# populationgenomics/cuKING

Hardware: AMD Instinct MI355X
Metric: sample-pairs/s (all-pairs KING) (higher is better)
Workload: dtype fp4 products, f32 accumulate (exact integers)

## Files before the change

### cuking_amd/_lib.py

```python
from __future__ import annotations

import ctypes as C
from pathlib import Path

PKG = Path(__file__).resolve().parent
LIB_PATH = PKG / "libcuking_amd.so"

OK = 0
ERR_INVALID_ARGUMENT = 1
ERR_FAILED_PRECONDITION = 2
ERR_RESOURCE_EXHAUSTED = 3
ERR_OUT_OF_MEMORY = 4
ERR_DEVICE = 5

KERNEL_TILED = 0
KERNEL_STREAM = 1

KIN_UPPER = 0
KIN_SYMMETRIC = 1

KIN_BINS_MAX = 4096
REL_THRESHOLDS_MAX = 8
REL_NO_BAND = 0xFFFFFFFF

# ... 108 lines not shown
    "cuking_kin_best_key": (_u64, [_f32, _u32]),
    "cuking_kin_best_decode": (_u32, [_u64, C.POINTER(_f32), C.POINTER(_u32)]),
    "cuking_compute_kin_summary": (_int, [_vp, _SM, _u32, _vp, _BINS, _vp, _vp, _vp]),
    "cuking_compute_kin_summary_tiles": (_int, [_vp, _SM, _u32, _vp, _u64, _u64, _BINS, _vp,
                                                _vp, _vp]),
    "cuking_rel_band": (_u32, [C.POINTER(_f32), _u32, _f32]),
    "cuking_compute_relative_counts": (_int, [_vp, _SM, _u32, _vp, C.POINTER(_f32), _u32, _vp,
                                              _vp]),
    "cuking_compute_relative_counts_tiles": (_int, [_vp, _SM, _u32, _vp, _u64, _u64,
                                                    C.POINTER(_f32), _u32, _vp, _vp]),
    "cuking_unrelated_key": (_u64, [_f32, _u32]),
    "cuking_unrelated_set_host": (_int, [_vp, _u64, _u32, _f32, _vp, _vp, _vp]),
    "cuking_unrelated_set": (_int, [_vp, _vp, _u64, _u32, _f32, _vp, _vp, _vp, C.POINTER(_u32),
                                    _vp]),
    "cuking_site_counts": (_int, [_vp, _vp, _u32, _u32, _vp, _vp]),
    "cuking_sample_counts": (_int, [_vp, _vp, _u32, _u32, _u32, _vp, _vp]),
    "cuking_site_mask_host": (_int, [_vp, _u32, _u32, C.POINTER(CSiteFilter), _vp, _vp,
                                     C.POINTER(_u32)]),
    "cuking_compact_sites_host": (_int, [_vp, _u32, _u32, _vp, _u32, _vp, _u32]),
    "cuking_compact_sites": (_int, [_vp, _vp, _u32, _u32, _vp, _u32, _vp, _u32, _vp]),
    "cuking_ld_site_words": (_u32, [_u32]),
    "cuking_ld_priority": (_f32, [_vp]),
    "cuking_transpose_sites_host": (_int, [_vp, _u32, _u32, _u32, _vp, _u32]),
    "cuking_transpose_sites": (_int, [_vp, _vp, _u32, _u32, _u32, _vp, _u32, _vp]),
    "cuking_ld_edges_host": (_int, [_vp, _u32, _u32, _u32, _f32, _vp, _vp, _u64,
                                    C.POINTER(_u64)]),
    "cuking_ld_edges": (_int, [_vp, _vp, _u32, _u32, _u32, _f32, _vp, _vp, _u64,
                               C.POINTER(_u64), _vp]),
    "cuking_geno_matmul_host": (_int, [_vp, _u32, _u32, _u32, _vp, _int, _vp, _u32, _u32, _vp,
                                       _u32]),
# ... 89 lines not shown
```

### cuking_amd/build.py

```python
from __future__ import annotations

import argparse
import os
import shutil
import subprocess
import sys
from pathlib import Path

PKG = Path(__file__).resolve().parent
ROOT = PKG.parent
CSRC = PKG / "csrc"
HOST = PKG / "host"
INCLUDE = ROOT / "include"

LIB_PATH = PKG / "libcuking_amd.so"
CLI_PATH = PKG / "bin" / "cuking"
LIB_FLAGS_PATH = PKG / "libcuking_amd.flags"

HIP_SOURCES = ["king_abi.hip", "king_kernels.hip", "king_mfma.hip", "king_filter.hip",
               "king_sort.hip", "king_prune.hip", "king_bed.hip", "king_site_qc.hip",
               "king_ld.hip", "king_geno.hip", "king_pcrelate.hip",
               "king_pcrelate_records.hip", "king_pcrelate_pairs.hip", "king_ibd.hip",
               "king_ibd_scan.hip", "king_mendel.hip", "synth.hip"]
HOST_ABI_SOURCES = ["king_host.cc"]
# ... 38 lines not shown
    cwd = PKG / "build_tmp"
    cwd.mkdir(exist_ok=True)
    cmd += ["-save-temps"]
    if save_temps:
        cmd += ["-Rpass-analysis=kernel-resource-usage"]
        subprocess.run(cmd, check=True, cwd=str(cwd))
    else:
        with open(cwd / "build.log", "w") as log:
            r = subprocess.run(cmd, cwd=str(cwd), stdout=log, stderr=subprocess.STDOUT)
        if r.returncode != 0:
            sys.stderr.write((cwd / "build.log").read_text()[-8000:])
            raise subprocess.CalledProcessError(r.returncode, cmd)
    problems = check_mfma_loops(cwd / "king_mfma-hip-amdgcn-amd-amdhsa-gfx950.s")
    problems += check_filter_loop(cwd / "king_filter-hip-amdgcn-amd-amdhsa-gfx950.s")
    problems += check_no_scratch(cwd / "king_bed-hip-amdgcn-amd-amdhsa-gfx950.s", "pack_bed_kernel")
    for kernel in ("site_counts_kernel", "sample_counts_kernel", "compact_sites_kernel"):
        problems += check_no_scratch(cwd / "king_site_qc-hip-amdgcn-amd-amdhsa-gfx950.s", kernel)
    for kernel in ("transpose_sites_kernel", "ld_edges_kernel"):
        problems += check_no_scratch(cwd / "king_ld-hip-amdgcn-amd-amdhsa-gfx950.s", kernel)
    problems += check_no_scratch(cwd / "king_geno-hip-amdgcn-amd-amdhsa-gfx950.s",
                                 "geno_matmul_kernel")
    problems += check_no_scratch(cwd / "king_pcrelate-hip-amdgcn-amd-amdhsa-gfx950.s",
                                 "pcrelate_matrix_kernel")
    problems += check_no_scratch(cwd / "king_pcrelate_records-hip-amdgcn-amd-amdhsa-gfx950.s",
                                 "pcrelate_records_kernel")
    problems += check_no_scratch(cwd / "king_pcrelate_pairs-hip-amdgcn-amd-amdhsa-gfx950.s",
                                 "pcrelate_pairs_kernel")
    for kernel in ("ibd_pairs_kernel", "roh_samples_kernel"):
        problems += check_no_scratch(cwd / "king_ibd-hip-amdgcn-amd-amdhsa-gfx950.s", kernel)
    problems += check_no_scratch(cwd / "king_ibd_scan-hip-amdgcn-amd-amdhsa-gfx950.s",
# ... 128 lines not shown
```

### cuking_amd/csrc/king_abi.hip

```cpp
#include <hip/hip_runtime.h>

#include <algorithm>
#include <cstdio>
#include <cstdlib>
#include <cstring>
#include <vector>

#include "king_common.h"
#include "king_geno.h"
#include "king_host.h"
#include "king_ibd.h"
#include "king_kin_summary.h"
#include "king_ld.h"
#include "king_site_qc.h"
#include "king_unrelated.h"

using namespace cuking;

namespace {

#define HIP_TRY(expr)                                                      \
  do {                                                                     \
    const hipError_t _e = (expr);                                          \
    if (_e != hipSuccess) {                                                \
// ... 89 lines not shown
    DeviceBuf prune, sites, record_count, ibd_groups, site_order;
  };
  std::vector<StreamScratch> scratch;
  unsigned long long filter_totals_retired[kNumTotals] = {};
  uint32_t filter_quadrant_cap = kFilterQuadrantCap;
  uint32_t filter_cand_cap = kFilterCandCap;
  uint32_t filter_split_min_steps = 8;
  int filter_check0 = 1, filter_check1 = 1, filter_check_emit = (int)kCheckEmitCap;
  int filter_rotate = 1;
  uint32_t filter_rotate_min_steps = 128;
  uint32_t filter_rotate_min_tiles = 2048;
  int filter_sort = 1;
  bool filter_lazy_codes = true;
  int filter_site_order = -1;
  uint32_t filter_site_order_min_tiles = (uint32_t)kSiteOrderMinTiles;
  SiteOrderForecast order_forecast = {0, 0, false};
  float order_sigma = 0.f;
  void *sort_temp = nullptr;
  size_t sort_temp_bytes = 0;

  void *synth_tables = nullptr;
  size_t synth_tables_bytes = 0;
  hipStream_t synth_stream = nullptr;
  hipEvent_t synth_done = nullptr;

  struct Prepared {
    bool valid = false;
    cuking_submatrix sm = {0, 0, 0, 0};
    uint32_t words_per_sample = 0;
    int variant = -1;
// ... 476 lines not shown
  const uint32_t all_tiles = (geo.s_stride + 63) / 64;
  const uint32_t t_end = s_tile_end < all_tiles ? s_tile_end : all_tiles;
  cuking_ctx::Prepared &pr = ctx->prepared;
  const bool new_prefix = !same_tile_space(ctx->prefix_for, tiles);
  const uint32_t num_stored = geo.diag ? geo.num_rows : geo.num_rows + geo.num_cols;
  SiteOrderScratch order_layout = {};
  bool order_wanted = false;
  if (filter_call && !dense_order && v.layout == kLayoutNibbleStats && ctx->filter_site_order != 0 &&
      s_tile_begin == 0 && t_end == all_tiles) {
    order_layout = site_order_scratch(num_stored, words_per_sample);
    order_wanted = order_layout.bytes != 0 &&
                 (ctx->filter_site_order >= 1 ||
                  (total_tiles(tiles) >= ctx->filter_site_order_min_tiles &&
                   geo.k_words / 8 >= filter_check_min_steps()));
  }
  const bool same = same_block(pr, sm, words_per_sample, variant, v.tile, d_bit_sets) &&
                    pr.dense_order == dense_order && pr.order_wanted == order_wanted &&
                    !(pr.site_order && pr.order_thr != kin_threshold);
  if (ctx->reuse_prepared && same && !new_prefix) {
    bool all_there = true;
    for (uint32_t t = s_tile_begin; t < t_end && all_there; ++t) all_there = pr.tiles[t] != 0;
    if (all_there) {
      ++ctx->conversions_skipped;
      if (v.layout == kLayoutNibbleStats && need_codes && !pr.codes)
        return convert_codes_now(ctx, geo, words_per_sample, d_bit_sets, stream);
      return CUKING_OK;
    }
  }
  const bool other_stream = pr.ordered_valid && pr.ordered_on != stream;
  bool must_wait = new_prefix && !ctx->readers.empty();
// ... 49 lines not shown
                                order_layout, d_curve, stream));
      SiteCurve curve;
      HIP_TRY(hipMemcpyAsync(&curve, d_curve, sizeof curve, hipMemcpyDeviceToHost, stream));
      ++ctx->host_syncs;
      HIP_TRY(hipStreamSynchronize(stream));
      const SiteOrderForecast f = site_order_forecast(curve, num_stored, geo.k_words, kin_threshold);
      ctx->order_forecast = f;
      ctx->order_sigma = curve.sigma;
      site_order = ctx->filter_site_order >= 1 ||
                   (!f.verdict_first && f.order64 != 0 &&
                    (f.stored64 == 0 || f.order64 + kSiteOrderMinGain <= f.stored64));
      pr.order_thr = kin_threshold;
      pr.order_no_left = site_order ? 0u : kSiteOrderNoTrust;
    }
    pr.site_order = site_order;
    if (site_order) {
      cuking_ctx::StreamScratch *e = stream_entry(ctx, stream);
      HIP_TRY(launch_site_permute(d_bit_sets, num_stored, words_per_sample, e->site_order.p,
                                  order_layout, stream));
      layout_bits = reinterpret_cast<const uint64_t *>(static_cast<const uint8_t *>(e->site_order.p) +
                                                       order_layout.permuted);
    }
    HIP_TRY(launch_sample_stats(layout_bits, words_per_sample, geo, ctx->planes, sb, se, stream));
    HIP_TRY(launch_sample_order(geo, words_per_sample, ctx->planes, sb, se,
                                !dense_order &&
                                    (ctx->filter_sort == 2 || (ctx->filter_sort == 1 && whole)),
                                ctx->sort_temp, ctx->sort_temp_bytes, stream));
    HIP_TRY(launch_prepare_nibbles(codes && !site_order, true, layout_bits, words_per_sample, geo,
                                   ctx->planes, plane_perm(ctx->planes, geo), s_tile_begin, t_end,
                                   nullptr, nullptr, stream));
    if (codes && site_order)
      HIP_TRY(launch_prepare_nibbles(true, false, d_bit_sets, words_per_sample, geo, ctx->planes,
                                     plane_perm(ctx->planes, geo), s_tile_begin, t_end, nullptr,
                                     nullptr, stream));
    if (!codes) {
      pr.codes = false;
    } else if (!pr.codes) {
      st = convert_codes_now(ctx, geo, words_per_sample, d_bit_sets, stream);
// ... 88 lines not shown

enum : uint8_t {
  kInvalidatesLayout = 1,
  kResizesSlabs = 2,
};

struct Option {
  const char *key;
  int64_t lo, hi;
  const char *error;
  uint32_t error_arg;
  uint8_t effects;
  int64_t (*get)(const cuking_ctx *);
  void (*set)(cuking_ctx *, int64_t);
  int64_t hole = INT64_MIN;
};

#define CTX_FIELD(f)                                                     \
  [](const cuking_ctx *c) -> int64_t { return (int64_t)c->f; },          \
  [](cuking_ctx *c, int64_t v) { c->f = (decltype(c->f))v; }

const Option kOptions[] = {
    {"variant", 0, kNumTiledVariants - 1, "variant outside [0, %u)", kNumTiledVariants, 0,
     CTX_FIELD(variant)},
    {"band_rows", 0, 64, "band_rows outside [0, 64]", 0, 0, CTX_FIELD(band_rows)},
    {"counts_mode", -1, 1, "counts_mode outside [-1, 1]", 0, 0, CTX_FIELD(counts_mode)},
    {"split_wgs", 0, 4096, "split_wgs outside [0, 4096]", 0, kResizesSlabs, CTX_FIELD(split_wgs)},
    {"xcd_swizzle", 0, 2, "xcd_swizzle outside [0, 2]", 0, 0, CTX_FIELD(xcd_swizzle)},
    {"dyn_tail_tiles", 0, 0x7FFFFFFF, "dyn_tail_tiles outside [0, 2^31)", 0, 0,
     CTX_FIELD(dyn_tail_tiles)},
    {"reuse_prepared", 0, 1, "reuse_prepared outside [0, 1]", 0, 0, CTX_FIELD(reuse_prepared)},
    {"filter_sort", 0, 2, "filter_sort outside [0, 2]", 0, kInvalidatesLayout,
     CTX_FIELD(filter_sort)},
    {"filter_lazy_codes", 0, 1, "filter_lazy_codes outside [0, 1]", 0, kInvalidatesLayout,
     CTX_FIELD(filter_lazy_codes)},
    {"filter_site_order", -1, 2, "filter_site_order outside [-1, 2]", 0, kInvalidatesLayout,
     CTX_FIELD(filter_site_order)},
    {"filter_site_order_min_tiles", 0, 1 << 30, "filter_site_order_min_tiles outside [0, 2^30]",
     0, kInvalidatesLayout, CTX_FIELD(filter_site_order_min_tiles)},
    {"filter_check0", 0, 2, "filter_check0 outside [0, 2]", 0, 0, CTX_FIELD(filter_check0)},
    {"filter_check1", 0, 1 + kNumCheckShares, "filter_check1 outside {0, 1, 3 .. %u}",
     1 + kNumCheckShares, 0, CTX_FIELD(filter_check1), 2},
    {"filter_check_emit", 0, 255, "filter_check_emit outside [0, 255]", 0, 0,
     CTX_FIELD(filter_check_emit)},
    {"filter_rotate", 0, 2 + kNumPhases, "filter_rotate outside [0, %u]", 2 + kNumPhases, 0,
     CTX_FIELD(filter_rotate)},
    {"filter_rotate_min_steps", 1, 1 << 20, "filter_rotate_min_steps outside [1, 2^20]", 0, 0,
     CTX_FIELD(filter_rotate_min_steps)},
    {"filter_rotate_min_tiles", 0, 1 << 30, "filter_rotate_min_tiles outside [0, 2^30]", 0, 0,
     CTX_FIELD(filter_rotate_min_tiles)},
    {"filter_quadrant_cap", 0, 16384, "filter_quadrant_cap outside [0, 16384]", 0, 0,
     CTX_FIELD(filter_quadrant_cap)},
    {"filter_cand_cap", 0, kFilterCandCap, "filter_cand_cap outside [0, %u]", kFilterCandCap, 0,
     CTX_FIELD(filter_cand_cap)},
// ... 122 lines not shown

cuking_status cuking_ctx_set_kernel(cuking_ctx *ctx, cuking_kernel kernel) {
  if (ctx == nullptr) return cuking_fail(CUKING_ERR_INVALID_ARGUMENT, "null context");
  if (kernel != CUKING_KERNEL_TILED && kernel != CUKING_KERNEL_STREAM)
    return cuking_fail(CUKING_ERR_INVALID_ARGUMENT, "unknown kernel %d", (int)kernel);
  ctx->kernel = kernel;
  return CUKING_OK;
}

cuking_status cuking_ctx_set_option(cuking_ctx *ctx, const char *key,
                                    int64_t value) {
  if (ctx == nullptr || key == nullptr)
    return cuking_fail(CUKING_ERR_INVALID_ARGUMENT, "null argument");
  const Option *o = find_option(key);
  if (o == nullptr) return cuking_fail(CUKING_ERR_INVALID_ARGUMENT, "unknown option %s", key);
  if (value < o->lo || value > o->hi || value == o->hole)
    return cuking_fail(CUKING_ERR_INVALID_ARGUMENT, o->error, o->error_arg);
  if ((o->effects & kResizesSlabs) && value != o->get(ctx)) {
    HIP_TRY(hipDeviceSynchronize());
    for (auto &e : ctx->scratch) free_split_slab(e);
  }
  o->set(ctx, value);
  if (o->effects & kInvalidatesLayout) ctx->prepared.valid = false;
  return CUKING_OK;
}

cuking_status cuking_device_alloc(cuking_ctx *ctx, size_t bytes, void **d_ptr) {
  BIND_OR_RETURN(ctx);
  if (d_ptr == nullptr) return cuking_fail(CUKING_ERR_INVALID_ARGUMENT, "null out pointer");
  *d_ptr = nullptr;
  if (bytes == 0) return CUKING_OK;
// ... 732 lines not shown

cuking_status cuking_site_counts(cuking_ctx *ctx, const uint64_t *d_bit_set,
                                 uint32_t num_stored, uint32_t words_per_sample,
                                 uint32_t *d_counts, void *stream) {
  if (ctx == nullptr) return cuking_fail(CUKING_ERR_INVALID_ARGUMENT, "null context");
  cuking_status st = cuking_check_counts_args("site counts", d_bit_set, num_stored,
                                              words_per_sample, d_counts);
  if (st != CUKING_OK) return st;
  if (num_stored == 0) return CUKING_OK;
  BIND_OR_RETURN(ctx);
  HIP_TRY(launch_site_counts(d_bit_set, num_stored, words_per_sample, d_counts,
                             (hipStream_t)stream));
  return CUKING_OK;
}

cuking_status cuking_sample_counts(cuking_ctx *ctx, const uint64_t *d_bit_set,
                                   uint32_t num_stored, uint32_t words_per_sample,
                                   uint32_t num_sites, uint32_t *d_counts, void *stream) {
  if (ctx == nullptr) return cuking_fail(CUKING_ERR_INVALID_ARGUMENT, "null context");
  cuking_status st = cuking_check_counts_args("sample counts", d_bit_set, num_stored,
                                              words_per_sample, d_counts);
  if (st != CUKING_OK) return st;
  if (cuking_words_per_sample(num_sites) != words_per_sample)
    return cuking_fail(CUKING_ERR_INVALID_ARGUMENT,
                       "sample counts: %u sites need %u words per sample, not %u", num_sites,
                       cuking_words_per_sample(num_sites), words_per_sample);
  if (num_stored == 0) return CUKING_OK;
  BIND_OR_RETURN(ctx);
  HIP_TRY(launch_sample_counts(d_bit_set, num_stored, words_per_sample, num_sites, d_counts,
                               (hipStream_t)stream));
// ... 406 lines not shown
```

### cuking_amd/csrc/king_common.h

```cpp
#ifndef CUKING_AMD_KING_COMMON_H_
#define CUKING_AMD_KING_COMMON_H_

#include <hip/hip_runtime.h>
#include <stdint.h>

#include "cuking_amd.h"
#include "king_launch_plan.h"
#include "king_submatrix.h"

namespace cuking {

constexpr uint32_t kLayoutWord = 0;
constexpr uint32_t kLayoutQuad = 1;
constexpr uint32_t kLayoutNibble = 2;
constexpr uint32_t kLayoutNibbleStats = 3;

struct PlaneGeometry {
  uint32_t num_rows, num_cols;
  uint32_t rows_padded, cols_padded;
  uint32_t col_base;
  uint32_t s_stride;
  uint32_t k_words;
  uint32_t diag;
};
// ... 267 lines not shown
hipError_t launch_mfma_list(const TiledArgs &args, const uint2 *list, const uint32_t *count,
                            uint32_t cap, uint32_t grid, hipStream_t stream);
hipError_t launch_mfma_gated(const TiledArgs &args, uint64_t num_units, const uint32_t *gate,
                             const uint8_t *skip_tiles, uint64_t skip_base, uint32_t grid,
                             hipStream_t stream);
hipError_t launch_filter(const TiledArgs &args, const LaunchSwitches &sw, uint64_t num_tiles,
                         hipStream_t stream);
inline void to_quadrants(TiledArgs *a, uint64_t *num_units) {
  a->quad = 1;
  a->tile_begin *= 4;
  *num_units *= 4;
}
hipError_t launch_sample_stats(const uint64_t *d_bit_sets, uint32_t words_per_sample,
                               const PlaneGeometry &geo, uint4 *d_planes, uint32_t s_begin,
                               uint32_t s_end, hipStream_t stream);
void set_filter_check_min_steps(uint32_t steps);
uint32_t filter_check_min_steps();
size_t sort_temp_bytes_for(uint32_t n);
hipError_t launch_sample_order(const PlaneGeometry &geo, uint32_t words_per_sample,
                               uint4 *d_planes, uint32_t s_begin, uint32_t s_end, bool sort,
                               void *sort_temp, size_t sort_temp_bytes, hipStream_t stream);
struct SiteOrderScratch {
  size_t counts, keys, vals, sort_temp, sort_temp_bytes, permuted, bytes;
};
SiteOrderScratch site_order_scratch(uint32_t num_stored, uint32_t words_per_sample);
hipError_t launch_site_order(const uint64_t *d_bit_sets, uint32_t num_stored,
                             uint32_t words_per_sample, const PlaneGeometry &geo, void *d_scratch,
                             const SiteOrderScratch &layout, SiteCurve *d_curve,
                             hipStream_t stream);
hipError_t launch_site_permute(const uint64_t *d_bit_sets, uint32_t num_stored,
                               uint32_t words_per_sample, void *d_scratch,
                               const SiteOrderScratch &layout, hipStream_t stream);
struct SiteOrderForecast {
  uint32_t stored64, order64;
  bool verdict_first;
};
SiteOrderForecast site_order_forecast(const SiteCurve &curve, uint32_t num_stored,
                                      uint32_t k_words, float thr);
hipError_t launch_prepare_nibbles(bool codes, bool t2, const uint64_t *d_bit_sets,
                                  uint32_t words_per_sample, const PlaneGeometry &geo,
                                  uint4 *d_planes, const uint32_t *perm, uint32_t s_tile_begin,
                                  uint32_t s_tile_end, const uint32_t *gate,
                                  const uint32_t *ready, hipStream_t stream);
hipError_t launch_mark_codes_ready(const uint32_t *gate, uint32_t *ready, hipStream_t stream);
size_t mfma_split_scratch_bytes(uint32_t wgs);
size_t mfma_split_counter_bytes(uint32_t wgs);

// ... 124 lines not shown
```

### cuking_amd/csrc/king_filter.hip

```cpp
#include <hip/hip_runtime.h>
#include <stdio.h>

#include <atomic>
#include <stdlib.h>

#include "king_common.h"
#include "king_device.h"
#include "king_kin_summary.h"

#pragma clang diagnostic ignored "-Winline-asm"

namespace cuking {

namespace {

typedef int v8i __attribute__((ext_vector_type(8)));
typedef float v16f __attribute__((ext_vector_type(16)));

constexpr int kT = (int)kFilterTile;
constexpr int kUnits = 2;
constexpr int kStages = 5;
constexpr int kSliceU4 = kT;
constexpr int kStageU4 = 2 * 2 * kUnits * kSliceU4;
constexpr int kStageReqs = 4 * kUnits;
// ... 946 lines not shown
        atomicAdd(a.rel_counts + (size_t)off_j * a.rel_num + band, 1u);
      }
    }
  }
}

}

static std::atomic<uint32_t> g_check_min_steps{64};
void set_filter_check_min_steps(uint32_t steps) { g_check_min_steps.store(steps); }
uint32_t filter_check_min_steps() { return g_check_min_steps.load(); }

hipError_t launch_sample_stats(const uint64_t *d_bit_sets, uint32_t words_per_sample,
                               const PlaneGeometry &geo, uint4 *d_planes, uint32_t s_begin,
                               uint32_t s_end, hipStream_t stream) {
  if (s_end > geo.s_stride) s_end = geo.s_stride;
  if (s_begin >= s_end) return hipSuccess;
  float2 *stats = plane_tmp_stats(d_planes, geo);
  float *prefix = plane_tmp_prefix(d_planes, geo);
  unsigned long long *sums = const_cast<unsigned long long *>(plane_cohort_sums(d_planes, geo));
  uint32_t *steps = const_cast<uint32_t *>(plane_check_steps(d_planes, geo));
  CheckWords cw;
  const uint32_t all_steps = geo.k_words / 8;
  if (all_steps > kStatsMaxSteps) return hipErrorInvalidValue;
  for (uint32_t k = 0; k < kNumCheckShares; ++k)
    cw.w[k] = check_step_of(all_steps, k, g_check_min_steps.load());
  sample_stats_kernel<<<dim3((s_end - s_begin + 3) / 4), dim3(256), 0, stream>>>(
      d_bit_sets, words_per_sample, geo, stats, prefix, sums, steps, cw, s_begin, s_end);
  return hipGetLastError();
}

hipError_t launch_filter(const TiledArgs &args, const LaunchSwitches &switches, uint64_t num_tiles,
                         hipStream_t stream) {
  if ((uint64_t)args.geo.k_words * 32 > kMfmaN4MaxSites || args.filter_ctrl == nullptr ||
      args.cand_list == nullptr || args.dense_list == nullptr || args.sample_stats == nullptr)
    return hipErrorInvalidValue;
// ... 68 lines not shown
```

### cuking_amd/csrc/king_sort.hip

```cpp
#include <hip/hip_runtime.h>

#include <hipcub/hipcub.hpp>

#include "king_common.h"

namespace cuking {

namespace {

__global__ void sort_keys_kernel(const float2 *__restrict__ tmp_stats, uint32_t begin, uint32_t n,
                                 float stored_sites, uint32_t *__restrict__ keys,
                                 uint32_t *__restrict__ vals) {
  const uint32_t p = blockIdx.x * blockDim.x + threadIdx.x;
  if (p >= n) return;
  const float2 st = tmp_stats[begin + p];
  const float missing = 0.5f * (stored_sites - st.y - st.x);
  uint32_t key = (uint32_t)(missing * 64.f / stored_sites);
  keys[p] = key > 255u ? 255u : key;
  vals[p] = begin + p;
}

__global__ void identity_order_kernel(uint32_t begin, uint32_t n, uint32_t *__restrict__ vals) {
  const uint32_t p = blockIdx.x * blockDim.x + threadIdx.x;
  if (p < n) vals[p] = begin + p;
// ... 214 lines not shown
            om[g] = bm;
          }
        }
      }
    }
    if (w0 + lane < P) {
#pragma unroll
      for (int g = 0; g < G; ++g) {
        if (s0 + g >= num_stored) continue;
        uint64_t *dst = out + (uint64_t)(s0 + g) * words_per_sample + w0 + lane;
        dst[0] = oh[g];
        dst[P] = om[g];
      }
    }
  }
}

size_t up256(size_t x) { return (x + 255) / 256 * 256; }

int weight_bits(uint32_t n) {
  int b = 1;
  while (b < 32 && (1ull << b) <= n) ++b;
  return 2 * b + 2 < 64 ? 2 * b + 2 : 64;
}

}

SiteOrderScratch site_order_scratch(uint32_t num_stored, uint32_t words_per_sample) {
  SiteOrderScratch l = {};
  const uint32_t P = words_per_sample / 2;
// ... 37 lines not shown
  e = hipGetLastError();
  if (e != hipSuccess) return e;
  size_t temp = l.sort_temp_bytes;
  e = hipcub::DeviceRadixSort::SortPairsDescending(base + l.sort_temp, temp, keys_in, keys_out,
                                                   vals_in, vals_out, (int)sites, 0,
                                                   weight_bits(num_stored), stream);
  if (e != hipSuccess) return e;
  site_curve_kernel<<<dim3(kNumPhases), dim3(256), 0, stream>>>(counts, vals_out, sites,
                                                                geo.k_words / 8, phase_w, phase_v);
  e = hipGetLastError();
  if (e != hipSuccess) return e;
  site_curve_scan_kernel<<<dim3(1), dim3(64), 0, stream>>>(phase_w, phase_v, d_curve);
  return hipGetLastError();
}

hipError_t launch_site_permute(const uint64_t *d_bit_sets, uint32_t num_stored,
                               uint32_t words_per_sample, void *d_scratch,
                               const SiteOrderScratch &l, hipStream_t stream) {
  if (l.bytes == 0 || d_scratch == nullptr) return hipErrorInvalidValue;
  const uint32_t P = words_per_sample / 2, sites = P * 64;
  uint8_t *base = static_cast<uint8_t *>(d_scratch);
  const uint32_t *vals_out = reinterpret_cast<const uint32_t *>(base + l.vals) + sites;
  uint64_t *permuted = reinterpret_cast<uint64_t *>(base + l.permuted);
  const uint32_t groups2 = (num_stored + 1) / 2;
  if ((size_t)P * 32 <= kOrderLdsBytes)
    permute_sites_kernel<2><<<dim3(groups2), dim3(256), P * 32, stream>>>(
        d_bit_sets, permuted, vals_out, num_stored, words_per_sample);
  else
    permute_sites_kernel<1><<<dim3(num_stored), dim3(256), P * 16, stream>>>(
        d_bit_sets, permuted, vals_out, num_stored, words_per_sample);
  return hipGetLastError();
}

SiteOrderForecast site_order_forecast(const SiteCurve &c, uint32_t num_stored, uint32_t k_words,
                                      float thr) {
  SiteOrderForecast f = {0, 0, false};
  const float sites = 32.f * (float)k_words, ns = (float)num_stored;
  if (!(ns > 0.f && c.het_calls != 0)) return f;
  const float m = (float)c.missing_calls / (ns * sites), h = (float)c.het_calls / (ns * sites);
  const float mean = m * (1.f + m / (2.f * h * (1.f - m))), sigma = 1.f / sqrtf(sites);
  f.verdict_first = mean - 4.f * sigma > thr;
  const float k_lin = mean + 4.6f * sigma + 0.003f, k_ord = mean + 4.6f * c.sigma + 0.003f;
  if (k_lin < 0.5f) {
    const float f64 = 64.f * (1.f - 2.f * thr) / (1.f - 2.f * k_lin);
    if (f64 <= 62.f) f.stored64 = f64 > 32.f ? (uint32_t)ceilf(f64) : 32u;
  }
// ... 10 lines not shown
```

### include/cuking_amd.h

```cpp
#ifndef CUKING_AMD_H_
#define CUKING_AMD_H_

#include <stddef.h>
#include <stdint.h>

#ifdef __cplusplus
extern "C" {
#endif

#define CUKING_ABI_VERSION 2

typedef enum cuking_status {
  CUKING_OK = 0,
  CUKING_ERR_INVALID_ARGUMENT = 1,
  CUKING_ERR_FAILED_PRECONDITION = 2,
  CUKING_ERR_RESOURCE_EXHAUSTED = 3,
  CUKING_ERR_OUT_OF_MEMORY = 4,
  CUKING_ERR_DEVICE = 5
} cuking_status;

typedef struct cuking_submatrix {
  uint32_t i_begin, i_end;
  uint32_t j_begin, j_end;
} cuking_submatrix;
// ... 414 lines not shown
                                       cuking_mendel_trio *out, uint64_t *error_bits);
cuking_status cuking_mendel_trios(cuking_ctx *ctx, const uint64_t *d_bits, uint32_t num_stored,
                                  uint32_t words_per_sample, uint32_t num_sites,
                                  const uint32_t *d_trios, uint64_t num_trios,
                                  cuking_mendel_trio *d_out, uint64_t *d_error_bits,
                                  void *stream);
cuking_status cuking_mendel_site_counts_host(const uint64_t *error_bits, uint64_t num_trios,
                                             uint32_t plane_words, uint32_t *counts);
cuking_status cuking_mendel_site_counts(cuking_ctx *ctx, const uint64_t *d_error_bits,
                                        uint64_t num_trios, uint32_t plane_words,
                                        uint32_t *d_counts, void *stream);

void cuking_sort_results(cuking_result *results, size_t num_results);


cuking_status cuking_timing_enable(cuking_ctx *ctx, int enabled);
cuking_status cuking_timing_reset(cuking_ctx *ctx);
cuking_status cuking_timing_collect(cuking_ctx *ctx, double *king_ms,
                                    uint64_t *king_launches, double *prepare_ms,
                                    uint64_t *prepare_launches);

cuking_status cuking_clock_probe(cuking_ctx *ctx, uint64_t microseconds,
                                 uint64_t *d_ticks, void *stream);


cuking_status cuking_synth_bitset(cuking_ctx *ctx, uint64_t seed,
                                  const uint32_t *d_kind, const uint32_t *d_pa,
                                  const uint32_t *d_pb, uint32_t sample_begin,
                                  uint32_t sample_end, uint32_t num_sites,
                                  uint32_t words_per_sample,
// ... 16 lines not shown
```

Baseline: 43.89 billion.

## Add byte/nibble-wide LDS site gather with fused per-sample statistics

```diff
diff --git a/cuking_amd/_lib.py b/cuking_amd/_lib.py
--- a/cuking_amd/_lib.py
+++ b/cuking_amd/_lib.py
@@ -146,6 +146,8 @@
     "cuking_unrelated_set": (_int, [_vp, _vp, _u64, _u32, _f32, _vp, _vp, _vp, C.POINTER(_u32),
                                     _vp]),
     "cuking_site_counts": (_int, [_vp, _vp, _u32, _u32, _vp, _vp]),
+    "cuking_test_site_gather": (_int, [_vp, _vp, _u32, _u32, _vp, _int, _vp, _int, _vp, _u64,
+                                       _vp, _vp]),
     "cuking_sample_counts": (_int, [_vp, _vp, _u32, _u32, _u32, _vp, _vp]),
     "cuking_site_mask_host": (_int, [_vp, _u32, _u32, C.POINTER(CSiteFilter), _vp, _vp,
                                      C.POINTER(_u32)]),
diff --git a/cuking_amd/build.py b/cuking_amd/build.py
--- a/cuking_amd/build.py
+++ b/cuking_amd/build.py
@@ -76,6 +76,8 @@
     problems = check_mfma_loops(cwd / "king_mfma-hip-amdgcn-amd-amdhsa-gfx950.s")
     problems += check_filter_loop(cwd / "king_filter-hip-amdgcn-amd-amdhsa-gfx950.s")
     problems += check_no_scratch(cwd / "king_bed-hip-amdgcn-amd-amdhsa-gfx950.s", "pack_bed_kernel")
+    problems += check_no_scratch(cwd / "king_sort-hip-amdgcn-amd-amdhsa-gfx950.s",
+                                 "gather_sites_kernel")
     for kernel in ("site_counts_kernel", "sample_counts_kernel", "compact_sites_kernel"):
         problems += check_no_scratch(cwd / "king_site_qc-hip-amdgcn-amd-amdhsa-gfx950.s", kernel)
     for kernel in ("transpose_sites_kernel", "ld_edges_kernel"):
diff --git a/cuking_amd/csrc/king_abi.hip b/cuking_amd/csrc/king_abi.hip
--- a/cuking_amd/csrc/king_abi.hip
+++ b/cuking_amd/csrc/king_abi.hip
@@ -127,6 +127,7 @@
   bool filter_lazy_codes = true;
   int filter_site_order = -1;
   uint32_t filter_site_order_min_tiles = (uint32_t)kSiteOrderMinTiles;
+  int filter_site_gather = -1;
   SiteOrderForecast order_forecast = {0, 0, false};
   float order_sigma = 0.f;
   void *sort_temp = nullptr;
@@ -633,6 +634,11 @@
                   (total_tiles(tiles) >= ctx->filter_site_order_min_tiles &&
                    geo.k_words / 8 >= filter_check_min_steps()));
   }
+  const int site_gather = site_gather_pick(ctx->filter_site_gather, words_per_sample);
+  if (order_wanted && site_gather < 0)
+    return cuking_fail(CUKING_ERR_INVALID_ARGUMENT,
+                       "filter_site_gather %d: %u words per sample do not fit the gather's LDS",
+                       ctx->filter_site_gather, words_per_sample);
   const bool same = same_block(pr, sm, words_per_sample, variant, v.tile, d_bit_sets) &&
                     pr.dense_order == dense_order && pr.order_wanted == order_wanted &&
                     !(pr.site_order && pr.order_thr != kin_threshold);
@@ -712,14 +718,18 @@
       pr.order_no_left = site_order ? 0u : kSiteOrderNoTrust;
     }
     pr.site_order = site_order;
+    const bool fused_stats = site_order && site_gather > 0 && geo.diag != 0;
     if (site_order) {
       cuking_ctx::StreamScratch *e = stream_entry(ctx, stream);
+      const SiteGatherStats fused = {stats_arrays(geo, ctx->planes), geo, se};
       HIP_TRY(launch_site_permute(d_bit_sets, num_stored, words_per_sample, e->site_order.p,
-                                  order_layout, stream));
+                                  order_layout, site_gather, fused_stats ? &fused : nullptr,
+                                  stream));
       layout_bits = reinterpret_cast<const uint64_t *>(static_cast<const uint8_t *>(e->site_order.p) +
                                                        order_layout.permuted);
     }
-    HIP_TRY(launch_sample_stats(layout_bits, words_per_sample, geo, ctx->planes, sb, se, stream));
+    HIP_TRY(launch_sample_stats(layout_bits, words_per_sample, geo, ctx->planes,
+                                fused_stats ? num_stored : sb, se, stream));
     HIP_TRY(launch_sample_order(geo, words_per_sample, ctx->planes, sb, se,
                                 !dense_order &&
                                     (ctx->filter_sort == 2 || (ctx->filter_sort == 1 && whole)),
@@ -838,6 +848,7 @@
   int64_t (*get)(const cuking_ctx *);
   void (*set)(cuking_ctx *, int64_t);
   int64_t hole = INT64_MIN;
+  bool (*valid)(int64_t) = nullptr;
 };
 
 #define CTX_FIELD(f)                                                     \
@@ -862,6 +873,9 @@
      CTX_FIELD(filter_site_order)},
     {"filter_site_order_min_tiles", 0, 1 << 30, "filter_site_order_min_tiles outside [0, 2^30]",
      0, kInvalidatesLayout, CTX_FIELD(filter_site_order_min_tiles)},
+    {"filter_site_gather", -1, 4, "filter_site_gather outside {-1, 0, 2, 4}", 0,
+     kInvalidatesLayout, CTX_FIELD(filter_site_gather), INT64_MIN,
+     [](int64_t v) { return v == -1 || (v & 1) == 0; }},
     {"filter_check0", 0, 2, "filter_check0 outside [0, 2]", 0, 0, CTX_FIELD(filter_check0)},
     {"filter_check1", 0, 1 + kNumCheckShares, "filter_check1 outside {0, 1, 3 .. %u}",
      1 + kNumCheckShares, 0, CTX_FIELD(filter_check1), 2},
@@ -1014,7 +1028,7 @@
     return cuking_fail(CUKING_ERR_INVALID_ARGUMENT, "null argument");
   const Option *o = find_option(key);
   if (o == nullptr) return cuking_fail(CUKING_ERR_INVALID_ARGUMENT, "unknown option %s", key);
-  if (value < o->lo || value > o->hi || value == o->hole)
+  if (value < o->lo || value > o->hi || value == o->hole || (o->valid && !o->valid(value)))
     return cuking_fail(CUKING_ERR_INVALID_ARGUMENT, o->error, o->error_arg);
   if ((o->effects & kResizesSlabs) && value != o->get(ctx)) {
     HIP_TRY(hipDeviceSynchronize());
@@ -1777,6 +1791,62 @@
   return CUKING_OK;
 }
 
+cuking_status cuking_test_site_gather(cuking_ctx *ctx, const uint64_t *d_bit_set,
+                                      uint32_t num_stored, uint32_t words_per_sample,
+                                      const uint32_t *d_order, int gather, uint64_t *d_permuted,
+                                      int stats, void *d_stats, uint64_t stats_bytes,
+                                      uint64_t *layout, void *stream) {
+  if (ctx == nullptr) return cuking_fail(CUKING_ERR_INVALID_ARGUMENT, "null context");
+  if (d_bit_set == nullptr || d_order == nullptr || d_permuted == nullptr)
+    return cuking_fail(CUKING_ERR_INVALID_ARGUMENT, "site gather: null pointer");
+  if (num_stored == 0 || words_per_sample < 2)
+    return cuking_fail(CUKING_ERR_INVALID_ARGUMENT, "site gather: no samples or no plane words");
+  if ((gather != 0 && gather != 2 && gather != 4) ||
+      site_gather_pick(gather, words_per_sample) != gather)
+    return cuking_fail(CUKING_ERR_INVALID_ARGUMENT,
+                       "site gather: form %d does not serve %u words per sample", gather,
+                       words_per_sample);
+  if (stats < 0 || stats > 2 || (stats == 1 && gather == 0))
+    return cuking_fail(CUKING_ERR_INVALID_ARGUMENT,
+                       "site gather: statistics %d with form %d (0 none, 1 inside the byte-wide "
+                       "gather, 2 the separate kernel)", stats, gather);
+  cuking_submatrix sm;
+  cuking_status status = cuking_submatrix_init(&sm, num_stored, 1, 0);
+  if (status != CUKING_OK) return status;
+  const PlaneGeometry geo = make_geometry(sm, words_per_sample, tiled_variant(7));
+  const uint64_t off_cum = (uint64_t)geo.s_stride * sizeof(float2);
+  const uint64_t off_sums = off_cum + (uint64_t)geo.s_stride * (kNumCum + 1) * sizeof(float);
+  const uint64_t off_steps = off_sums + 64, bytes = off_steps + 64;
+  if (layout != nullptr) {
+    layout[0] = geo.s_stride;
+    layout[1] = off_cum;
+    layout[2] = off_sums;
+    layout[3] = off_steps;
+    layout[4] = bytes;
+  }
+  if (stats != 0 && (d_stats == nullptr || stats_bytes < bytes))
+    return cuking_fail(CUKING_ERR_INVALID_ARGUMENT,
+                       "site gather: the statistics need %llu bytes", (unsigned long long)bytes);
+  BIND_OR_RETURN(ctx);
+  uint8_t *base = static_cast<uint8_t *>(d_stats);
+  SiteGatherStats fused = {};
+  if (stats != 0) {
+    fused.to = {reinterpret_cast<float2 *>(base), reinterpret_cast<float *>(base + off_cum),
+                reinterpret_cast<unsigned long long *>(base + off_sums),
+                reinterpret_cast<uint32_t *>(base + off_steps)};
+    fused.geo = geo;
+    fused.s_end = geo.s_stride;
+    HIP_TRY(hipMemsetAsync(base + off_sums, 0, 64, (hipStream_t)stream));
+  }
+  HIP_TRY(launch_site_gather(d_bit_set, num_stored, words_per_sample, d_order, d_permuted, gather,
+                             stats == 1 ? &fused : nullptr, (hipStream_t)stream));
+  if (stats != 0)
+    HIP_TRY(launch_sample_stats_to(d_permuted, words_per_sample, geo, fused.to,
+                                   stats == 1 ? num_stored : 0, geo.s_stride,
+                                   (hipStream_t)stream));
+  return CUKING_OK;
+}
+
 cuking_status cuking_sample_counts(cuking_ctx *ctx, const uint64_t *d_bit_set,
                                    uint32_t num_stored, uint32_t words_per_sample,
                                    uint32_t num_sites, uint32_t *d_counts, void *stream) {
diff --git a/cuking_amd/csrc/king_common.h b/cuking_amd/csrc/king_common.h
--- a/cuking_amd/csrc/king_common.h
+++ b/cuking_amd/csrc/king_common.h
@@ -305,6 +305,20 @@
 hipError_t launch_sample_stats(const uint64_t *d_bit_sets, uint32_t words_per_sample,
                                const PlaneGeometry &geo, uint4 *d_planes, uint32_t s_begin,
                                uint32_t s_end, hipStream_t stream);
+struct SampleStatsArrays {
+  float2 *stats;
+  float *cum;
+  unsigned long long *sums;
+  uint32_t *steps;
+};
+inline SampleStatsArrays stats_arrays(const PlaneGeometry &geo, uint4 *d_planes) {
+  return {plane_tmp_stats(d_planes, geo), plane_tmp_prefix(d_planes, geo),
+          const_cast<unsigned long long *>(plane_cohort_sums(d_planes, geo)),
+          const_cast<uint32_t *>(plane_check_steps(d_planes, geo))};
+}
+hipError_t launch_sample_stats_to(const uint64_t *d_bit_sets, uint32_t words_per_sample,
+                                  const PlaneGeometry &geo, const SampleStatsArrays &to,
+                                  uint32_t s_begin, uint32_t s_end, hipStream_t stream);
 void set_filter_check_min_steps(uint32_t steps);
 uint32_t filter_check_min_steps();
 size_t sort_temp_bytes_for(uint32_t n);
@@ -319,9 +333,20 @@
                              uint32_t words_per_sample, const PlaneGeometry &geo, void *d_scratch,
                              const SiteOrderScratch &layout, SiteCurve *d_curve,
                              hipStream_t stream);
+int site_gather_pick(int option, uint32_t words_per_sample);
+struct SiteGatherStats {
+  SampleStatsArrays to;
+  PlaneGeometry geo;
+  uint32_t s_end;
+};
 hipError_t launch_site_permute(const uint64_t *d_bit_sets, uint32_t num_stored,
                                uint32_t words_per_sample, void *d_scratch,
-                               const SiteOrderScratch &layout, hipStream_t stream);
+                               const SiteOrderScratch &layout, int gather,
+                               const SiteGatherStats *fused, hipStream_t stream);
+hipError_t launch_site_gather(const uint64_t *d_bit_sets, uint32_t num_stored,
+                              uint32_t words_per_sample, const uint32_t *d_order,
+                              uint64_t *d_permuted, int gather, const SiteGatherStats *fused,
+                              hipStream_t stream);
 struct SiteOrderForecast {
   uint32_t stored64, order64;
   bool verdict_first;
diff --git a/cuking_amd/csrc/king_filter.hip b/cuking_amd/csrc/king_filter.hip
--- a/cuking_amd/csrc/king_filter.hip
+++ b/cuking_amd/csrc/king_filter.hip
@@ -984,12 +984,19 @@
 hipError_t launch_sample_stats(const uint64_t *d_bit_sets, uint32_t words_per_sample,
                                const PlaneGeometry &geo, uint4 *d_planes, uint32_t s_begin,
                                uint32_t s_end, hipStream_t stream) {
+  return launch_sample_stats_to(d_bit_sets, words_per_sample, geo, stats_arrays(geo, d_planes),
+                                s_begin, s_end, stream);
+}
+
+hipError_t launch_sample_stats_to(const uint64_t *d_bit_sets, uint32_t words_per_sample,
+                                  const PlaneGeometry &geo, const SampleStatsArrays &to,
+                                  uint32_t s_begin, uint32_t s_end, hipStream_t stream) {
   if (s_end > geo.s_stride) s_end = geo.s_stride;
   if (s_begin >= s_end) return hipSuccess;
-  float2 *stats = plane_tmp_stats(d_planes, geo);
-  float *prefix = plane_tmp_prefix(d_planes, geo);
-  unsigned long long *sums = const_cast<unsigned long long *>(plane_cohort_sums(d_planes, geo));
-  uint32_t *steps = const_cast<uint32_t *>(plane_check_steps(d_planes, geo));
+  float2 *stats = to.stats;
+  float *prefix = to.cum;
+  unsigned long long *sums = to.sums;
+  uint32_t *steps = to.steps;
   CheckWords cw;
   const uint32_t all_steps = geo.k_words / 8;
   if (all_steps > kStatsMaxSteps) return hipErrorInvalidValue;
diff --git a/cuking_amd/csrc/king_site_gather.h b/cuking_amd/csrc/king_site_gather.h
--- /dev/null
+++ b/cuking_amd/csrc/king_site_gather.h
@@ -0,0 +1,64 @@
+#ifndef CUKING_KING_SITE_GATHER_H_
+#define CUKING_KING_SITE_GATHER_H_
+
+#include <stdint.h>
+
+#if defined(__HIPCC__) || defined(__CUDACC__)
+#define CUKING_GATHER_HD __host__ __device__ __forceinline__
+#else
+#define CUKING_GATHER_HD inline
+#endif
+
+namespace cuking {
+
+constexpr uint32_t kGatherBatch = 16;
+constexpr uint32_t kGatherTileBytes = kGatherBatch * 64;
+
+CUKING_GATHER_HD uint32_t gather_field_bit(uint32_t g, uint32_t plane) { return 2 * g + plane; }
+
+CUKING_GATHER_HD uint32_t gather_site_bytes(uint32_t group, uint32_t plane_words) {
+  return group == 4 ? 64 * plane_words : 32 * plane_words;
+}
+
+CUKING_GATHER_HD uint64_t transpose8x8(uint64_t x) {
+  uint64_t t = (x ^ (x >> 7)) & 0x00AA00AA00AA00AAull;
+  x ^= t ^ (t << 7);
+  t = (x ^ (x >> 14)) & 0x0000CCCC0000CCCCull;
+  x ^= t ^ (t << 14);
+  t = (x ^ (x >> 28)) & 0x00000000F0F0F0F0ull;
+  x ^= t ^ (t << 28);
+  return x;
+}
+
+CUKING_GATHER_HD uint64_t gather_interleave8(const uint64_t fields[8], uint32_t b) {
+  uint64_t x = 0;
+#pragma unroll
+  for (uint32_t f = 0; f < 8; ++f) x |= ((fields[f] >> (8 * b)) & 0xFFull) << (8 * f);
+  return transpose8x8(x);
+}
+
+CUKING_GATHER_HD uint32_t gather_pack_nibbles(uint64_t x) {
+  x = (x | (x >> 4)) & 0x00FF00FF00FF00FFull;
+  x = (x | (x >> 8)) & 0x0000FFFF0000FFFFull;
+  return (uint32_t)(x | (x >> 16));
+}
+
+CUKING_GATHER_HD uint32_t gather_byte_index(uint32_t group, uint32_t src) {
+  return group == 4 ? src : src >> 1;
+}
+CUKING_GATHER_HD uint32_t gather_field_of(uint32_t group, uint32_t src, uint32_t byte) {
+  return group == 4 ? byte : (byte >> (4 * (src & 1))) & 0xFu;
+}
+
+CUKING_GATHER_HD uint64_t gather_assemble8(uint64_t fields_of_sites) {
+  return transpose8x8(fields_of_sites);
+}
+CUKING_GATHER_HD uint32_t gather_out_byte(uint32_t f, uint32_t k, uint32_t b) {
+  return (f * kGatherBatch + k) * 8 + b;
+}
+CUKING_GATHER_HD uint32_t gather_out_field(uint32_t i) { return i / kGatherBatch; }
+CUKING_GATHER_HD uint32_t gather_out_word(uint32_t i) { return i % kGatherBatch; }
+
+}
+
+#endif
diff --git a/cuking_amd/csrc/king_sort.hip b/cuking_amd/csrc/king_sort.hip
--- a/cuking_amd/csrc/king_sort.hip
+++ b/cuking_amd/csrc/king_sort.hip
@@ -3,6 +3,8 @@
 #include <hipcub/hipcub.hpp>
 
 #include "king_common.h"
+#include "king_device.h"
+#include "king_site_gather.h"
 
 namespace cuking {
 
@@ -252,6 +254,216 @@
       }
     }
   }
+}
+
+constexpr uint32_t kGatherLdsMax = 160 * 1024;
+
+__device__ __forceinline__ void wave_lds_order() {
+  __builtin_amdgcn_fence(__ATOMIC_ACQ_REL, "wavefront");
+  __builtin_amdgcn_wave_barrier();
+}
+
+struct GatherStatsArgs {
+  float2 *stats;
+  float *cum;
+  unsigned long long *sums;
+  uint32_t *steps_out;
+  uint32_t s_stride, all_steps, stats_grid;
+  uint32_t steps[kNumCheckShares];
+};
+constexpr uint32_t kGatherStatsBytes = 4 * (kNumPhases + 4) * 4;
+
+template <int G, bool STATS>
+__global__ __launch_bounds__(1024) void gather_sites_kernel(
+    const uint64_t *__restrict__ bits, uint64_t *__restrict__ out,
+    const uint32_t *__restrict__ order, uint32_t num_stored, uint32_t words_per_sample,
+    GatherStatsArgs st) {
+  extern __shared__ uint4 gather_lds[];
+  static_assert(G == 2 || G == 4, "a nibble or a byte per site");
+  static_assert(kGatherBatch % 8 == 0 && (2 * G * kGatherBatch) % 64 == 0, "whole rounds");
+  static_assert(kGatherBatch == 16, "the statistics: 16 lanes per sample");
+  const uint32_t P = words_per_sample / 2;
+  const uint32_t s0 = blockIdx.x * G;
+  const uint32_t lane = threadIdx.x & 63, wave = threadIdx.x >> 6, waves = blockDim.x >> 6;
+  uint8_t *site = reinterpret_cast<uint8_t *>(gather_lds);
+  uint8_t *tile = site + ((gather_site_bytes(G, P) + 15u) & ~15u) + wave * kGatherTileBytes;
+  int32_t *phase_sum = reinterpret_cast<int32_t *>(site + ((gather_site_bytes(G, P) + 15u) & ~15u) +
+                                                   waves * kGatherTileBytes);
+  int32_t *totals = phase_sum + G * kNumPhases;
+  if (STATS) {
+    for (uint32_t i = threadIdx.x; i < G * (kNumPhases + 4); i += blockDim.x) phase_sum[i] = 0;
+    if (blockIdx.x == 0) {
+#pragma unroll
+      for (uint32_t k = 0; k < kNumCheckShares; ++k)
+        if (threadIdx.x == k) st.steps_out[k] = st.steps[k];
+    }
+  }
+  int32_t yc = 0, mc = 0, hc = 0, sa = 0;
+
+  const uint64_t *het[G];
+#pragma unroll
+  for (int g = 0; g < G; ++g) {
+    const uint32_t s = s0 + g < num_stored ? s0 + g : num_stored - 1;
+    het[g] = bits + (uint64_t)s * words_per_sample;
+  }
+  for (uint32_t w = threadIdx.x; w < P; w += blockDim.x) {
+    uint64_t f[8] = {0, 0, 0, 0, 0, 0, 0, 0};
+#pragma unroll
+    for (int g = 0; g < G; ++g) {
+      f[gather_field_bit(g, 0)] = het[g][w];
+      f[gather_field_bit(g, 1)] = het[g][P + w];
+    }
+    if (G == 4) {
+      uint4 *dst = reinterpret_cast<uint4 *>(site + 64 * w);
+#pragma unroll
+      for (uint32_t b = 0; b < 8; b += 2) {
+        const uint64_t lo = gather_interleave8(f, b), hi = gather_interleave8(f, b + 1);
+        dst[b / 2] = make_uint4((uint32_t)lo, (uint32_t)(lo >> 32), (uint32_t)hi, (uint32_t)(hi >> 32));
+      }
+    } else {
+      uint4 *dst = reinterpret_cast<uint4 *>(site + 32 * w);
+#pragma unroll
+      for (uint32_t b = 0; b < 8; b += 4)
+        dst[b / 4] = make_uint4(gather_pack_nibbles(gather_interleave8(f, b)),
+                                gather_pack_nibbles(gather_interleave8(f, b + 1)),
+                                gather_pack_nibbles(gather_interleave8(f, b + 2)),
+                                gather_pack_nibbles(gather_interleave8(f, b + 3)));
+    }
+  }
+  __syncthreads();
+
+  constexpr uint32_t kRounds = kGatherBatch / 8;
+  constexpr uint32_t kOutRounds = 2 * G * kGatherBatch / 64;
+  uint64_t *tile64 = reinterpret_cast<uint64_t *>(tile);
+  const uint32_t last_site = 64 * P - 1;
+  for (uint32_t w0 = kGatherBatch * wave; w0 < P; w0 += kGatherBatch * waves) {
+    uint32_t src[kGatherBatch];
+#pragma unroll
+    for (uint32_t k = 0; k < kGatherBatch; ++k) {
+      const uint32_t W = w0 + k < P ? w0 + k : P - 1;
+      const uint32_t at = order[64 * W + lane];
+      src[k] = at < last_site ? at : last_site;
+    }
+    uint32_t field[kGatherBatch];
+#pragma unroll
+    for (uint32_t k = 0; k < kGatherBatch; ++k) field[k] = site[gather_byte_index(G, src[k])];
+#pragma unroll
+    for (uint32_t k = 0; k < kGatherBatch; ++k)
+      tile[64 * k + lane] = (uint8_t)gather_field_of(G, src[k], field[k]);
+    wave_lds_order();
+    uint64_t x[kRounds];
+#pragma unroll
+    for (uint32_t r = 0; r < kRounds; ++r) x[r] = tile64[64 * r + lane];
+    wave_lds_order();
+#pragma unroll
+    for (uint32_t r = 0; r < kRounds; ++r) {
+      const uint64_t y = gather_assemble8(x[r]);
+      const uint32_t k = 8 * r + (lane >> 3), b = lane & 7;
+#pragma unroll
+      for (uint32_t f = 0; f < 2 * G; ++f) tile[gather_out_byte(f, k, b)] = (uint8_t)(y >> (8 * f));
+    }
+    wave_lds_order();
+#pragma unroll
+    for (uint32_t r = 0; r < kOutRounds; ++r) {
+      const uint32_t i = 64 * r + lane, f = gather_out_field(i), k = gather_out_word(i);
+      const uint64_t word = tile64[i];
+      const uint32_t s = s0 + f / 2;
+      if (w0 + k < P && s < num_stored)
+        out[(uint64_t)s * words_per_sample + (f & 1) * P + w0 + k] = word;
+    }
+    if (STATS) {
+      const uint32_t g = (lane >> 4) & (G - 1), w = w0 + (lane & 15);
+      const bool in = (lane >> 4) < G && w < P;
+      const uint64_t h = in ? tile64[gather_field_bit(g, 0) * kGatherBatch + (lane & 15)] : 0ull;
+      const uint64_t v = in ? tile64[gather_field_bit(g, 1) * kGatherBatch + (lane & 15)] : 0ull;
+      const int32_t y = in ? __popcll(~h) : 0;
+      const int32_t m = __popcll(h & v);
+      yc += y;
+      mc += m;
+      hc += __popcll(h & ~v);
+      const uint64_t hom_a = in ? ~h & 0xFFFFFFFF00000000ull : 0ull;
+      const int32_t t_a = __popcll(hom_a & ~v) - __popcll(hom_a & v);
+      sa += t_a;
+      int32_t d = y - m + 2 * t_a;
+      d += __shfl_xor(d, 1);
+      d += __shfl_xor(d, 2);
+      if ((lane & 3) == 0 && in) {
+        const uint32_t x = (kNumPhases * ((w >> 2) + 1) - 1) / st.all_steps;
+        atomicAdd(&phase_sum[g * kNumPhases + (x < kNumPhases ? x : kNumPhases - 1)], d);
+      }
+    }
+    wave_lds_order();
+  }
+  if (!STATS) return;
+#pragma unroll
+  for (int off = 8; off > 0; off >>= 1) {
+    yc += __shfl_xor(yc, off);
+    mc += __shfl_xor(mc, off);
+    hc += __shfl_xor(hc, off);
+    sa += __shfl_xor(sa, off);
+  }
+  if ((lane & 15) == 0 && (lane >> 4) < G) {
+    int32_t *t = totals + 4 * (lane >> 4);
+    atomicAdd(t, yc);
+    atomicAdd(t + 1, mc);
+    atomicAdd(t + 2, hc);
+    atomicAdd(t + 3, sa);
+  }
+  __syncthreads();
+  const uint32_t ps = s0 + wave;
+  if (wave >= G || ps >= num_stored) return;
+  yc = totals[4 * wave];
+  mc = totals[4 * wave + 1];
+  hc = totals[4 * wave + 2];
+  sa = totals[4 * wave + 3];
+  static_assert(kNumPhases == 128, "two phases per lane");
+  const int32_t p0 = phase_sum[wave * kNumPhases + 2 * lane];
+  const int32_t p1 = phase_sum[wave * kNumPhases + 2 * lane + 1];
+  int32_t run = p0 + p1;
+#pragma unroll
+  for (int off = 1; off < 64; off <<= 1) {
+    const int32_t up = __shfl_up(run, off);
+    if ((int)lane >= off) run += up;
+  }
+  st.cum[(size_t)(2 * lane) * st.s_stride + ps] =
+      (float)(run - p1 + (int32_t)(128u * phase_step(st.all_steps, 2 * lane + 1)));
+  if (2 * lane + 1 < kNumCum)
+    st.cum[(size_t)(2 * lane + 1) * st.s_stride + ps] =
+        (float)(run + (int32_t)(128u * phase_step(st.all_steps, 2 * lane + 2)));
+  if (lane == 0) {
+    st.stats[ps] = make_float2((float)(yc - mc), (float)hc);
+    st.cum[(size_t)kNumCum * st.s_stride + ps] =
+        (float)(yc - mc + 2 * sa + (int32_t)(128u * st.all_steps));
+    if (((ps >> 2) & 15) == 0 || st.stats_grid < 64) {
+      relaxed_add(st.sums, 1ull);
+      relaxed_add(st.sums + 1, (unsigned long long)mc);
+      relaxed_add(st.sums + 2, (unsigned long long)hc);
+    }
+  }
+}
+
+uint32_t gather_lds_bytes(int group, uint32_t P, uint32_t threads) {
+  return ((gather_site_bytes((uint32_t)group, P) + 15u) & ~15u) + (threads / 64) * kGatherTileBytes +
+         kGatherStatsBytes;
+}
+uint32_t gather_threads(int group, uint32_t P) {
+  for (uint32_t threads = 1024; threads >= 512; threads /= 2)
+    if (gather_lds_bytes(group, P, threads) <= kGatherLdsMax) return threads;
+  return 0;
+}
+
+template <int G, bool STATS>
+hipError_t launch_gather_form(const uint64_t *d_bit_sets, uint32_t num_stored,
+                              uint32_t words_per_sample, const uint32_t *d_order,
+                              uint64_t *d_permuted, const GatherStatsArgs &st, hipStream_t stream) {
+  const uint32_t P = words_per_sample / 2, threads = gather_threads(G, P);
+  if (threads == 0) return hipErrorInvalidValue;
+  const hipError_t e = allow_dynamic_lds<gather_sites_kernel<G, STATS>>(kGatherLdsMax);
+  if (e != hipSuccess) return e;
+  gather_sites_kernel<G, STATS><<<dim3((num_stored + G - 1) / G), dim3(threads),
+                                  gather_lds_bytes(G, P, threads), stream>>>(
+      d_bit_sets, d_permuted, d_order, num_stored, words_per_sample, st);
+  return hipGetLastError();
 }
 
 size_t up256(size_t x) { return (x + 255) / 256 * 256; }
@@ -319,22 +531,70 @@
   return hipGetLastError();
 }
 
+int site_gather_pick(int option, uint32_t words_per_sample) {
+  const uint32_t P = words_per_sample / 2;
+  if (P == 0 || (size_t)P * 16 > kOrderLdsBytes) return option <= 0 ? 0 : -1;
+  if (option == 0) return 0;
+  if ((option == -1 || option == 4) && gather_threads(4, P) != 0) return 4;
+  if ((option == -1 || option == 2) && gather_threads(2, P) != 0) return 2;
+  return option == -1 ? 0 : -1;
+}
+
+hipError_t launch_site_gather(const uint64_t *d_bit_sets, uint32_t num_stored,
+                              uint32_t words_per_sample, const uint32_t *d_order,
+                              uint64_t *d_permuted, int gather, const SiteGatherStats *fused,
+                              hipStream_t stream) {
+  const uint32_t P = words_per_sample / 2;
+  if (num_stored == 0 || P == 0 || (size_t)P * 16 > kOrderLdsBytes) return hipErrorInvalidValue;
+  if (gather == 4 || gather == 2) {
+    GatherStatsArgs st = {};
+    if (fused != nullptr) {
+      const PlaneGeometry &geo = fused->geo;
+      const uint32_t s_end = fused->s_end < geo.s_stride ? fused->s_end : geo.s_stride;
+      if (!geo.diag || geo.num_rows != num_stored || s_end < num_stored || geo.k_words < 8)
+        return hipErrorInvalidValue;
+      st.stats = fused->to.stats;
+      st.cum = fused->to.cum;
+      st.sums = fused->to.sums;
+      st.steps_out = fused->to.steps;
+      st.s_stride = geo.s_stride;
+      st.all_steps = geo.k_words / 8;
+      st.stats_grid = (s_end + 3) / 4;
+      for (uint32_t k = 0; k < kNumCheckShares; ++k)
+        st.steps[k] = check_step_of(st.all_steps, k, filter_check_min_steps());
+    }
+    if (gather == 4)
+      return fused ? launch_gather_form<4, true>(d_bit_sets, num_stored, words_per_sample, d_order,
+                                                 d_permuted, st, stream)
+                   : launch_gather_form<4, false>(d_bit_sets, num_stored, words_per_sample,
+                                                  d_order, d_permuted, st, stream);
+    return fused ? launch_gather_form<2, true>(d_bit_sets, num_stored, words_per_sample, d_order,
+                                               d_permuted, st, stream)
+                 : launch_gather_form<2, false>(d_bit_sets, num_stored, words_per_sample, d_order,
+                                                d_permuted, st, stream);
+  }
+  if (gather != 0 || fused != nullptr) return hipErrorInvalidValue;
+  const uint32_t groups2 = (num_stored + 1) / 2;
+  if ((size_t)P * 32 <= kOrderLdsBytes)
+    permute_sites_kernel<2><<<dim3(groups2), dim3(256), P * 32, stream>>>(
+        d_bit_sets, d_permuted, d_order, num_stored, words_per_sample);
+  else
+    permute_sites_kernel<1><<<dim3(num_stored), dim3(256), P * 16, stream>>>(
+        d_bit_sets, d_permuted, d_order, num_stored, words_per_sample);
+  return hipGetLastError();
+}
+
 hipError_t launch_site_permute(const uint64_t *d_bit_sets, uint32_t num_stored,
                                uint32_t words_per_sample, void *d_scratch,
-                               const SiteOrderScratch &l, hipStream_t stream) {
+                               const SiteOrderScratch &l, int gather,
+                               const SiteGatherStats *fused, hipStream_t stream) {
   if (l.bytes == 0 || d_scratch == nullptr) return hipErrorInvalidValue;
-  const uint32_t P = words_per_sample / 2, sites = P * 64;
+  const uint32_t sites = (words_per_sample / 2) * 64;
   uint8_t *base = static_cast<uint8_t *>(d_scratch);
   const uint32_t *vals_out = reinterpret_cast<const uint32_t *>(base + l.vals) + sites;
   uint64_t *permuted = reinterpret_cast<uint64_t *>(base + l.permuted);
-  const uint32_t groups2 = (num_stored + 1) / 2;
-  if ((size_t)P * 32 <= kOrderLdsBytes)
-    permute_sites_kernel<2><<<dim3(groups2), dim3(256), P * 32, stream>>>(
-        d_bit_sets, permuted, vals_out, num_stored, words_per_sample);
-  else
-    permute_sites_kernel<1><<<dim3(num_stored), dim3(256), P * 16, stream>>>(
-        d_bit_sets, permuted, vals_out, num_stored, words_per_sample);
-  return hipGetLastError();
+  return launch_site_gather(d_bit_sets, num_stored, words_per_sample, vals_out, permuted, gather,
+                            fused, stream);
 }
 
 SiteOrderForecast site_order_forecast(const SiteCurve &c, uint32_t num_stored, uint32_t k_words,
diff --git a/include/cuking_amd.h b/include/cuking_amd.h
--- a/include/cuking_amd.h
+++ b/include/cuking_amd.h
@@ -452,6 +452,13 @@
 void cuking_sort_results(cuking_result *results, size_t num_results);
 
 
+cuking_status cuking_test_site_gather(cuking_ctx *ctx, const uint64_t *d_bit_set,
+                                      uint32_t num_stored, uint32_t words_per_sample,
+                                      const uint32_t *d_order, int gather, uint64_t *d_permuted,
+                                      int stats, void *d_stats, uint64_t stats_bytes,
+                                      uint64_t *layout, void *stream);
+
+
 cuking_status cuking_timing_enable(cuking_ctx *ctx, int enabled);
 cuking_status cuking_timing_reset(cuking_ctx *ctx);
 cuking_status cuking_timing_collect(cuking_ctx *ctx, double *king_ms,
```

After: 45.00 billion, median of 6. +2.5%, better.
